# Wallacoloo/libfriendship

Hardware: AMD Instinct MI355X
Metric: Msamples/sec at 4096 partials x 64 voices; achieved HBM GB/s vs roofline (higher is better)
Workload: dtype f32

## Files before the change

libfriendship_amd/build.py:

```python
import os
import subprocess
import sys

PKG_DIR = os.path.dirname(os.path.abspath(__file__))
CSRC = os.path.join(PKG_DIR, "csrc")
OUT = os.path.join(PKG_DIR, "libfriendship_hip.so")
SOURCES = ["engine.cpp", "graph.cpp", "match.cpp", "stage.cpp", "jit.cpp", "leafjit.cpp", "stagejit.cpp", "comm_rccl.cpp", "kernels.hip"]
HEADERS = ["bankplan.hpp", "graph.hpp", "kernels.hpp", "match.hpp", "stage.hpp", "jit.hpp", "leafshape.hpp", "comm.hpp", "range.hpp", os.path.join("..", "..", "include", "friendship_render.h"),
           os.path.join("..", "..", "include", "friendship_render_ext.h")]
FLAGS = ["--offload-arch=gfx950", "-O3", "-std=c++17", "-fPIC", "-shared", "-ffp-contract=off",
         "-fno-slp-vectorize", "-mllvm", "-simplifycfg-sink-common=false", "-Wall", "-Wextra"]


def needs_build():
    if not os.path.exists(OUT):
        return True
    t = os.path.getmtime(OUT)
    deps = [os.path.join(CSRC, s) for s in SOURCES + HEADERS] + [os.path.abspath(__file__)]
    return any(os.path.getmtime(d) > t for d in deps)


def build(force=False, verbose=True):
    if not force and not needs_build():
        return OUT
    hipcc = os.environ.get("HIPCC", "/opt/rocm/bin/hipcc")
    cmd = [hipcc] + FLAGS + ["-o", OUT] + [os.path.join(CSRC, s) for s in SOURCES] + ["-lhiprtc", "-ldl"]
    if verbose:
        print(" ".join(cmd), file=sys.stderr)
    subprocess.run(cmd, check=True)
    return OUT


if __name__ == "__main__":
    build(force="--force" in sys.argv)
```

libfriendship_amd/csrc/engine.cpp:

```cpp
#include <hip/hip_runtime_api.h>

#include <algorithm>
#include <cfloat>
#include <cmath>
#include <cstdio>
#include <cstdlib>
#include <chrono>
#include <cstring>
#include <sstream>
#include <string>
#include <unordered_set>
#include <vector>

#include "../../include/friendship_render_ext.h"
#include "bankplan.hpp"
#include "comm.hpp"
#include "graph.hpp"
#include "jit.hpp"
#include "kernels.hpp"
#include "match.hpp"
#include "stage.hpp"

namespace fr {

// ... 14 lines not shown
    DevBuf(DevBuf &&o) noexcept : p(o.p), bytes(o.bytes) { o.p = nullptr; o.bytes = 0; }
    DevBuf &operator=(DevBuf &&o) noexcept {
        if (this != &o) { release(); p = o.p; bytes = o.bytes; o.p = nullptr; o.bytes = 0; }
        return *this;
    }
    ~DevBuf() { release(); }
    void release() {
        if (p) (void)hipFree(p);
        p = nullptr;
        bytes = 0;
    }
    void ensure(size_t n) {
        if (n <= bytes) return;
        release();
        size_t want = std::max(n, (size_t)256);
        HIP_CHECK(hipMalloc(&p, want));
        bytes = want;
    }
    template <class T> T *as() const { return (T *)p; }
};

struct PinnedBuf {
    void *p = nullptr;
    void *dev = nullptr;
    size_t bytes = 0;
    PinnedBuf() = default;
    PinnedBuf(const PinnedBuf &) = delete;
    PinnedBuf &operator=(const PinnedBuf &) = delete;
    ~PinnedBuf() { if (p) (void)hipHostFree(p); }
    void ensure(size_t n) {
        if (n <= bytes) return;
        if (p) (void)hipHostFree(p);
        p = dev = nullptr;
        bytes = 0;
        size_t want = std::max(n, (size_t)4096);
        HIP_CHECK(hipHostMalloc(&p, want, hipHostMallocMapped));
        HIP_CHECK(hipHostGetDevicePointer(&dev, p, 0));
        bytes = want;
    }
    template <class T> T *as() const { return (T *)p; }
    template <class T> T *as_dev() const { return (T *)dev; }
};

struct InSlot {
    bool fed = false;
    uint64_t base = 0;
    uint64_t len = 0;
    DevBuf buf;
    uint64_t cap = 0;
};

struct BankStage {
    BankLaunch grp;
    DevBuf d_params, d_rows, d_groups, d_group_off;
    std::shared_ptr<JitKernel> jit;
};

struct Plan {
    bool valid = false;
    uint64_t version = 0;
    uint64_t shard_epoch = 0;
    bool jit_pending = false;
    uint64_t jit_epoch = 0;
    uint32_t n_slots = 0;
    uint32_t max_depth = 0;
    std::vector<BankStage> banks;
    StagedPlan sp;
    DevBuf d_instrs, d_progs;
    std::shared_ptr<JitKernel> stage_jit;
    DevBuf d_jprogs, d_ptab;
    uint32_t stage_shapes = 0;
    bool stage_valid = false;
    uint64_t stage_end = 0;
    std::vector<uint32_t> pull_rows;
    DevBuf d_split_dst;
    DevBuf d_nodes, d_roots;
    std::vector<uint32_t> input_slots;
    const FlatGraph *graph = nullptr;
    bool observed_stale = false;
    std::string json;
};

struct BankLaunchNote {
    BankPlan launch;
    uint32_t voices, partials;
    uint64_t frames;
    uint32_t log2_p, leaf_variant;
    bool row_flags;
};

constexpr size_t N_OPTIONS = 29;

struct TimerClass {
    double ms = 0;
    uint64_t launches = 0;
    std::vector<std::pair<hipEvent_t, hipEvent_t>> pending;
};

__attribute__((weak)) hipError_t launch_input_range(const RangeArgs &a, hipStream_t) {
    for (uint32_t r = 0; r < a.n_rows; ++r)
        for (uint32_t b = 0; b < a.blocks; ++b) {
            RangePart o{HUGE_VALF, -HUGE_VALF, 0, 0};
            for (uint64_t i = (uint64_t)b * RANGE_THREADS; i < a.len[r]; i += (uint64_t)a.blocks * RANGE_THREADS)
                for (uint64_t j = i; j < std::min<uint64_t>(i + RANGE_THREADS, a.len[r]); ++j) {
                    const float v = a.row[r][j];
                    if (v != v) o.flags |= RANGE_NAN;
                    else if (v == HUGE_VALF) o.flags |= RANGE_POS_INF;
// ... 682 lines not shown
        Plan p;
        p.version = mirror.version;
        p.shard_epoch = shard_epoch;
        p.n_slots = n_slots;
        const ShardSpec *shard_spec = sharded() ? &shard : nullptr;
        const auto t_begin = std::chrono::steady_clock::now();
        uint32_t lower_lo = 0, lower_hi = UINT32_MAX;
        if (sharded() && shard.mode == FR_SHARD_VOICES) my_rows(n_slots, lower_lo, lower_hi);
        const FlatGraph &fg = lowering.update(mirror, n_slots, lower_lo, lower_hi, sharded() && shard.mode == FR_SHARD_PARTIALS);
        const double lower_ms = std::chrono::duration<double, std::milli>(std::chrono::steady_clock::now() - t_begin).count();
        p.max_depth = fg.max_depth;
        bool use_jit = allow_jit && mode == FR_MODE_AUTO;
        if (!matcher || matcher_gen != lowering.generation()) {
            matcher.reset(new BankMatcher(fg, 20, use_jit, allow_template, track_from));
            matcher_gen = lowering.generation();
        }
        p.graph = &fg;
        const ObservedInputs obs = observed_inputs(st);
        const ObservedInputs *observed = delay_observed ? &obs : nullptr;
        p.sp = plan_stages(fg, mode == FR_MODE_AUTO, mode != FR_MODE_PULL, 20, use_jit, allow_template, matcher.get(), shard_spec, track_from, observed, track_history);
        std::vector<std::shared_ptr<JitKernel>> jits(p.sp.banks.size());
        p.jit_epoch = jit_cache.epoch();
        if (use_jit) {
            bool without = false;
            try {
                for (size_t i = 0; i < p.sp.banks.size(); ++i)
                    if (p.sp.banks[i].jit) {
                        const bool wait = p.sp.banks[i].tracks && jit_async_configured;
                        if (wait) jit_cache.set_async(false);
                        struct Restore { JitCache &c; bool on; ~Restore() { if (on) c.set_async(true); } } restore{jit_cache, wait};
                        jits[i] = jit_cache.get(p.sp.banks[i].shape, p.sp.banks[i].varying, p.sp.banks[i].literal_bits, p.sp.banks[i].alias);
                        if (!jits[i]) p.jit_pending = without = true;
                    }
            } catch (const Error &e) {
                jit_error = e.what();
                without = true;
                if (sharded() && shard.mode == FR_SHARD_PARTIALS && e.code != FR_ERR_UNSUPPORTED)
                    throw Error(FR_ERR_DEVICE, std::string("a kernel of the sharded plan could not be compiled on this rank (every rank must plan alike): ") + e.what());
            }
            if (without) {
                p.sp = plan_stages(fg, true, true, 20, false, true, nullptr, shard_spec, track_from, observed, track_history);
                jits.assign(p.sp.banks.size(), nullptr);
            }
        }
        size_t bank_i = 0;
        for (BankLaunch &bg : p.sp.banks) {
            BankStage bs;
            bs.jit = jits[bank_i++];
            bs.grp = std::move(bg);
            bs.d_params.ensure(bs.grp.params.size() * sizeof(float));
            bs.d_rows.ensure(bs.grp.rows.size() * sizeof(uint32_t));
            HIP_CHECK(hipMemcpyAsync(bs.d_params.p, bs.grp.params.data(), bs.grp.params.size() * sizeof(float), hipMemcpyHostToDevice, st));
            HIP_CHECK(hipMemcpyAsync(bs.d_rows.p, bs.grp.rows.data(), bs.grp.rows.size() * sizeof(uint32_t), hipMemcpyHostToDevice, st));
            if (bs.grp.general) {
                bs.d_groups.ensure(bs.grp.groups.size() * sizeof(uint32_t));
                bs.d_group_off.ensure(bs.grp.group_off.size() * sizeof(uint32_t));
                HIP_CHECK(hipMemcpyAsync(bs.d_groups.p, bs.grp.groups.data(), bs.grp.groups.size() * sizeof(uint32_t), hipMemcpyHostToDevice, st));
                HIP_CHECK(hipMemcpyAsync(bs.d_group_off.p, bs.grp.group_off.data(), bs.grp.group_off.size() * sizeof(uint32_t), hipMemcpyHostToDevice, st));
            }
            p.banks.push_back(std::move(bs));
        }
        p.sp.banks.clear();
        if (!p.sp.split.empty()) {
            std::vector<uint32_t> dst(p.sp.split.size());
            for (size_t i = 0; i < dst.size(); ++i) dst[i] = p.sp.split[i].dst | (p.sp.split[i].to_ring ? 0x80000000u : 0u);
            p.d_split_dst.ensure(dst.size() * sizeof(uint32_t));
            HIP_CHECK(hipMemcpyAsync(p.d_split_dst.p, dst.data(), dst.size() * sizeof(uint32_t), hipMemcpyHostToDevice, st));
            HIP_CHECK(hipStreamSynchronize(st));
        }
        if (!p.sp.progs.empty()) {
            p.d_instrs.ensure(p.sp.instrs.size() * sizeof(StageInstr));
            p.d_progs.ensure(p.sp.progs.size() * sizeof(StageProg));
            HIP_CHECK(hipMemcpyAsync(p.d_instrs.p, p.sp.instrs.data(), p.sp.instrs.size() * sizeof(StageInstr), hipMemcpyHostToDevice, st));
            HIP_CHECK(hipMemcpyAsync(p.d_progs.p, p.sp.progs.data(), p.sp.progs.size() * sizeof(StageProg), hipMemcpyHostToDevice, st));
            StageJitPlan sj;
            if (allow_jit && stage_jit_mode != 0 && plan_stage_jit(p.sp.progs, p.sp.instrs, 32, stage_jit_mode == 2, sj, mirror.sparkle,
                                                                              stage_block_env ? stage_block_env : (p.sp.feedback ? 16u : 1u),
                                                                              p.sp.feedback && p.sp.fused_carry_only)) {
                try {
                    p.stage_jit = jit_cache.get_source(sj.source, "jit_stage");
                    if (!p.stage_jit) {
                        p.jit_pending = true;
                        throw Error(FR_OK, "");
                    }
                    p.stage_shapes = sj.n_shapes;
                    p.d_jprogs.ensure(sj.progs.size() * sizeof(JitStageProg));
                    p.d_ptab.ensure(std::max<size_t>(sj.ptab.size(), 1) * sizeof(uint32_t));
                    HIP_CHECK(hipMemcpyAsync(p.d_jprogs.p, sj.progs.data(), sj.progs.size() * sizeof(JitStageProg), hipMemcpyHostToDevice, st));
                    if (!sj.ptab.empty())
                        HIP_CHECK(hipMemcpyAsync(p.d_ptab.p, sj.ptab.data(), sj.ptab.size() * sizeof(uint32_t), hipMemcpyHostToDevice, st));
                    HIP_CHECK(hipStreamSynchronize(st));
                } catch (const Error &e) {
                    if (e.code != FR_OK) jit_error = e.what();
                    p.stage_jit = nullptr;
                }
            }
        }
        p.pull_rows = p.sp.pull_rows;
        if (!p.pull_rows.empty()) {
            std::vector<DevNode> dn(fg.nodes.size());
            std::unordered_map<uint32_t, uint32_t> dense;
            for (size_t i = 0; i < dn.size(); ++i) {
                const FlatNode &n = fg.nodes[i];
                dn[i] = DevNode{n.op, n.a, n.b, n.depth};
                if (n.op == OP_INPUT) {
                    auto it = dense.emplace(n.a, (uint32_t)p.input_slots.size());
// ... 252 lines not shown
                        d_chunk_rows.ensure(seq.size() * sizeof(uint32_t));
                        HIP_CHECK(hipMemcpyAsync(d_chunk_rows.p, seq.data(), seq.size() * sizeof(uint32_t), hipMemcpyHostToDevice, st));
                        HIP_CHECK(hipStreamSynchronize(st));
                        d_chunk_rows_n = (uint32_t)seq.size();
                    }
                    j.out = d_chunk_ws.as<float>();
                    j.rows = d_chunk_rows.as<uint32_t>();
                    j.out_stride = blen;
                }
                if (bs.grp.tracks && trk) {
                    j.tracks = trk->p;
                    j.track_stride = trk->stride;
                    j.track_limit = trk->limit;
                } else if (bs.grp.tracks && call_tracks) {
                    if (b0 != idx || blen != n_times) throw Error(FR_ERR_UNSUPPORTED, "internal: a voice that reads tracks rendered over another window than the call's");
                    j.tracks = call_tracks;
                    j.track_stride = call_track_stride;
                    j.track_limit = (uint32_t)std::min<uint64_t>((uint64_t)track_from + call_track_rows, 0xFFFFFFFFull);
                }
                note_bank_launch(bp, bs, blen, flag_out.host_flags != nullptr);
                Scope sc(this, &t_bank, st);
                HIP_CHECK(launch_jit_bank(*bs.jit, j, st));
                if (bp.pieces_log2) {
                    ChunkCombineArgs c{};
                    c.ws = d_chunk_ws.as<float>();
                    c.out = a.out;
                    c.rows = a.rows;
                    c.out_stride = a.out_stride;
                    c.n_times = blen;
                    c.n_voices = a.n_voices;
                    c.log2_c = bp.pieces_log2;
                    HIP_CHECK(launch_chunk_combine(c, st));
                }
                sc.done();
                return;
            }
            a.voices_per_wave = bp.voices_per_wave;
            if (bs.grp.general) {
                a.groups = bs.d_groups.as<uint32_t>();
                a.group_off = bs.d_group_off.as<uint32_t>();
                a.hist_dst = nullptr;
                note_bank_launch(bp, bs, blen, flag_out.host_flags != nullptr);
                Scope sc(this, &t_bank, st);
                HIP_CHECK(launch_gbank(a, st));
                sc.done();
                return;
            }
            if (a.hist_dst && !bp.appends_rows) throw Error(FR_ERR_DEVICE, "internal: deferred history append on a short call");
            a.chunk_log2 = bp.chunk_log2;
            a.frames_per_lane = bp.frames_per_lane;
            a.waves_per_group = bp.waves_per_group;
            a.small_call = bp.small_call;
            a.leaf_variant = bank_tune.leaf_variant;
            if (flag_out.host_flags) {
                if (!bp.publishes_rows) throw Error(FR_ERR_DEVICE, "internal: a bank launch cannot publish row flags");
                a.host_flags = flag_out.host_flags;
                a.row_done = flag_out.row_done;
                a.flag_value = flag_out.value;
            }
            if (bp.ws_floats) {
                used_scratch = true;
                d_bank_ws.ensure(bp.ws_floats * sizeof(float));
                a.ws = d_bank_ws.as<float>();
                if (bp.ticket_words) {
                    const size_t need = bp.ticket_words * sizeof(uint32_t);
                    clean_counters(st);
                    if (need > d_tickets.bytes) {
                        d_tickets.ensure(need * 2);
                        HIP_CHECK(hipMemsetAsync(d_tickets.p, 0, d_tickets.bytes, st));
                    }
                    a.tickets = d_tickets.as<uint32_t>();
                }
            }
            note_bank_launch(bp, bs, blen, flag_out.host_flags != nullptr);
            Scope sc(this, &t_bank, st);
            HIP_CHECK(launch_bank(a, st));
            sc.done();
        };
        auto launch_bank_window = [&](BankStage &bs, uint64_t b0, uint64_t blen, int64_t tile_off) {
            if (!(bs.grp.tracks && tail_on() && tile_off < 0 && b0 < idx && b0 + blen == idx + n_times)) {
                launch_bank_part(bs, b0, blen, tile_off, nullptr);
                return;
            }
            for (uint64_t s0 = b0; s0 < idx;) {
                const uint64_t pos = s0 & (tail_cap - 1);
                const uint64_t len = std::min(idx - s0, tail_cap - pos);
                TrackSrc ts{nullptr, tail_cap, 0};
                if (tail_rows) {
                    ts.p = reinterpret_cast<const float *>(reinterpret_cast<uintptr_t>(d_tail.as<float>() + pos) - (uintptr_t)track_from * tail_cap * sizeof(float));
                    ts.limit = (uint32_t)std::min<uint64_t>((uint64_t)track_from + tail_rows, 0xFFFFFFFFull);
                }
                launch_bank_part(bs, s0, len, -1, &ts);
                s0 += len;
            }
            launch_bank_part(bs, idx, n_times, -1, nullptr);
        };
        std::vector<DevInput> tab(sp.input_slots.size());
        auto fill_tab = [&] {
            for (size_t i = 0; i < tab.size(); ++i) tab[i] = dev_input(sp.input_slots[i]);
            if (tab.size() > STAGE_INLINE_INPUTS) {
                d_in_table_stage.ensure(tab.size() * sizeof(DevInput));
                HIP_CHECK(hipMemcpyAsync(d_in_table_stage.p, tab.data(), tab.size() * sizeof(DevInput), hipMemcpyHostToDevice, st));
                HIP_CHECK(hipStreamSynchronize(st));
            }
        };
        uint64_t launch_stride = 0;
// ... 922 lines not shown
```

libfriendship_amd/csrc/kernels.hip:

```cpp
#include <hip/hip_runtime.h>

#include <cstdlib>
#include <type_traits>

#include "kernels.hpp"

#pragma clang fp contract(off)

namespace fr {

#ifdef FR_DIAG_STAMPS
__device__ unsigned long long *g_diag = nullptr;
#define FR_DIAG_MARK(slot)                                                                                                 \
    do {                                                                                                                   \
        if (g_diag && (threadIdx.x & 63u) == 0u) {                                                                         \
            unsigned long long v_ = __builtin_amdgcn_s_memrealtime();                                                      \
            if ((slot) == 3) v_ = (unsigned long long)__builtin_amdgcn_s_getreg(0xF804) | ((unsigned long long)(__builtin_amdgcn_s_getreg(0xF814) & 15u) << 32); \
            g_diag[((size_t)blockIdx.x * 16u + (threadIdx.x >> 6)) * 8u + (slot)] = v_;                                    \
            if ((slot) != 3) g_diag[((size_t)blockIdx.x * 16u + (threadIdx.x >> 6)) * 8u + 4u + (slot)] = __builtin_amdgcn_s_memtime(); \
        }                                                                                                                  \
    } while (0)
#else
#define FR_DIAG_MARK(slot) do { } while (0)
#endif
// ... 134 lines not shown
    float w[8], A[8];
};

__device__ __forceinline__ void load_group(ParamGroup &pg, const_f32_ptr p, uint32_t g) {
#pragma unroll
    for (int j = 0; j < 8; ++j) {
        pg.w[j] = p[(size_t)g * 16 + 2 * j];
        pg.A[j] = p[(size_t)g * 16 + 2 * j + 1];
    }
}

template <int I, int N, class Fn>
__device__ __forceinline__ void static_for(Fn &&fn) {
    if constexpr (I < N) {
        fn(std::integral_constant<int, I>{});
        static_for<I + 1, N>(fn);
    }
}

template <int F>
using Lvl = float (&)[F];
#define FR_LEVELS_DECL Lvl<F> s0, Lvl<F> s1, Lvl<F> s2, Lvl<F> s3, Lvl<F> s4, Lvl<F> s5, Lvl<F> s6, Lvl<F> s7, Lvl<F> s8
#define FR_LEVELS_PASS s0, s1, s2, s3, s4, s5, s6, s7, s8

template <int F, bool FAST, bool EXACT>
__device__ __forceinline__ void bank_group(const ParamGroup &pg, uint32_t g,
                                           const float (&t)[F], FR_LEVELS_DECL) {
    float v[F];
#pragma unroll
    for (int f = 0; f < F; ++f) {
        float l0 = bank_leaf<FAST, EXACT>(t[f], pg.w[0], pg.A[0]);
        float l1 = bank_leaf<FAST, EXACT>(t[f], pg.w[1], pg.A[1]);
        float l2 = bank_leaf<FAST, EXACT>(t[f], pg.w[2], pg.A[2]);
        float l3 = bank_leaf<FAST, EXACT>(t[f], pg.w[3], pg.A[3]);
        float l4 = bank_leaf<FAST, EXACT>(t[f], pg.w[4], pg.A[4]);
        float l5 = bank_leaf<FAST, EXACT>(t[f], pg.w[5], pg.A[5]);
        float l6 = bank_leaf<FAST, EXACT>(t[f], pg.w[6], pg.A[6]);
        float l7 = bank_leaf<FAST, EXACT>(t[f], pg.w[7], pg.A[7]);
        v[f] = ((l0 + l1) + (l2 + l3)) + ((l4 + l5) + (l6 + l7));
    }
#define FR_CARRY(K, SK)                                                    \
    if (((g >> K) & 1u) == 0u) {       \
        static_for<0, F>([&](auto f) { SK[f] = v[f]; });                   \
        return;                                                            \
    }                                                                      \
    static_for<0, F>([&](auto f) { v[f] = SK[f] + v[f]; });
    FR_CARRY(0u, s0) FR_CARRY(1u, s1) FR_CARRY(2u, s2) FR_CARRY(3u, s3) FR_CARRY(4u, s4)
    FR_CARRY(5u, s5) FR_CARRY(6u, s6) FR_CARRY(7u, s7)
#undef FR_CARRY
#pragma unroll
    for (int f = 0; f < F; ++f) s8[f] = v[f];
}

template <int F, bool FAST, bool EXACT>
__device__ __forceinline__ void bank_wave_sum(const float *params, uint32_t ngroups, uint32_t levels,
                                              const float (&t)[F], float (&res)[F], const ParamGroup *first = nullptr) {
    float s0[F], s1[F], s2[F], s3[F], s4[F], s5[F], s6[F], s7[F], s8[F];
#pragma unroll
    for (int f = 0; f < F; ++f)
        s0[f] = s1[f] = s2[f] = s3[f] = s4[f] = s5[f] = s6[f] = s7[f] = s8[f] = 0.0f;

    const_f32_ptr p = (const_f32_ptr)params;
    ParamGroup pa, pb;
    if (first) pa = *first;
    else load_group(pa, p, 0);
    for (uint32_t g = 0; g < ngroups; g += 2) {
        const bool has_b = g + 1 < ngroups;
        __builtin_amdgcn_s_waitcnt(0xC07F);
        if (has_b) load_group(pb, p, g + 1);
        bank_group<F, FAST, EXACT>(pa, g, t, FR_LEVELS_PASS);
        if (has_b) {
            __builtin_amdgcn_s_waitcnt(0xC07F);
            if (g + 2 < ngroups) load_group(pa, p, g + 2);
            bank_group<F, FAST, EXACT>(pb, g + 1, t, FR_LEVELS_PASS);
        }
    }
#pragma unroll
    for (int f = 0; f < F; ++f) {
        float r = s8[f];
        r = levels == 7u ? s7[f] : r;
        r = levels == 6u ? s6[f] : r;
        r = levels == 5u ? s5[f] : r;
        r = levels == 4u ? s4[f] : r;
        r = levels == 3u ? s3[f] : r;
        r = levels == 2u ? s2[f] : r;
        r = levels == 1u ? s1[f] : r;
        r = levels == 0u ? s0[f] : r;
        res[f] = r;
    }
}

__device__ __forceinline__ bool leaves_all_negzero(const float2 *params, uint32_t n, float t, uint32_t tid, uint32_t nthreads) {
    bool ok = true;
    for (uint32_t k = tid; k < n && ok; k += nthreads) {
        float2 p = params[k];
        ok = __float_as_uint(bank_leaf<false, true>(t, p.x, p.y)) == 0x80000000u;
    }
    return ok;
}

template <bool FAST>
__device__ __attribute__((noinline)) bool wave_leaves_all_negzero(const float *params, uint32_t ngroups, float t, unsigned long long lanes) {
    const_f32_ptr p = (const_f32_ptr)params;
    const bool wanted = (lanes >> (threadIdx.x & 63u)) & 1ull;
    uint32_t all_and = 0xFFFFFFFFu, all_or = 0u;
    ParamGroup pa, pb;
    load_group(pa, p, 0);
    auto fold = [&](const ParamGroup &pg) {
#pragma unroll
        for (int j = 0; j < 8; ++j) {
            uint32_t b = __float_as_uint(bank_leaf<FAST, true>(t, pg.w[j], pg.A[j]));
            all_and &= b;
            all_or |= b;
        }
    };
    for (uint32_t g = 0; g < ngroups; g += 2) {
        const bool has_b = g + 1 < ngroups;
        __builtin_amdgcn_s_waitcnt(0xC07F);
        if (has_b) load_group(pb, p, g + 1);
        fold(pa);
        if (has_b) {
            __builtin_amdgcn_s_waitcnt(0xC07F);
            if (g + 2 < ngroups) load_group(pa, p, g + 2);
            fold(pb);
        }
        if (__ballot(wanted && all_and == 0x80000000u && all_or == 0x80000000u) == 0ull) {
            __builtin_amdgcn_s_waitcnt(0xC07F);
            return false;
        }
    }
    return all_and == 0x80000000u && all_or == 0x80000000u;
}

__device__ __forceinline__ float bank_time(const BankArgs &a, uint64_t ti) {
    return (ti >= a.time_skip && ti - a.time_skip < a.time_valid) ? a.time[ti - a.time_skip] : 0.0f;
}
__device__ __forceinline__ uint64_t bank_out_index(const BankArgs &a, uint64_t ti) {
    return a.ring_mask ? ((a.ring_t0 + ti) & a.ring_mask) : ti;
}

template <int F, int MODE, int NW, bool FLAGS = false>
__global__ void __launch_bounds__(64 * NW) bank_kernel(BankArgs a, uint32_t tiles, uint32_t nblocks) {
    uint32_t b = blockIdx.x;
    uint32_t lid = (nblocks % 8u == 0u) ? (b % 8u) * (nblocks / 8u) + b / 8u : b;
    const uint32_t nchunks = 1u << (a.log2_p - a.chunk_log2);
    const uint32_t vc = lid / tiles;
    const uint32_t tile = lid - vc * tiles;
    const uint32_t voice = vc >> (a.log2_p - a.chunk_log2);
    const uint32_t chunk = vc & (nchunks - 1u);
    const uint32_t lane = threadIdx.x & 63u;
    const uint32_t wave = __builtin_amdgcn_readfirstlane(threadIdx.x >> 6);

    FR_DIAG_MARK(0);
    FR_DIAG_MARK(3);
    const uint64_t t0 = (uint64_t)tile * (64u * F);
    float t[F];
    bool nonneg = true;
#pragma unroll
    for (int f = 0; f < F; ++f) {
        uint64_t ti = t0 + (uint32_t)f * 64u + lane;
        t[f] = bank_time(a, ti);
        nonneg = nonneg && (t[f] >= 0.0f) && (t[f] <= 4294967296.0f);
        if (a.hist_dst && vc == 0u && wave == 0u && ti < a.time_valid) a.hist_dst[ti] = t[f];
    }
    const bool fast = a.fast_ok && __all(nonneg);

    const uint32_t Pc = 1u << a.chunk_log2;
    const uint32_t Pw = Pc / NW;
    const float2 *cparams = a.params + ((size_t)voice << a.log2_p) + (size_t)chunk * Pc;
    const float *params = (const float *)(cparams + (size_t)wave * Pw);
    const uint32_t ngroups = Pw >> 3;
    const uint32_t levels = a.chunk_log2 - 3u - (NW == 8 ? 3u : NW == 4 ? 2u : NW == 2 ? 1u : 0u);

    float res[F];
    constexpr bool EXACT = (MODE == 0);
    if (fast) bank_wave_sum<F, true, EXACT>(params, ngroups, levels, t, res);
    else bank_wave_sum<F, false, EXACT>(params, ngroups, levels, t, res);
    FR_DIAG_MARK(1);

    __shared__ float sm[NW][F][64];
    __shared__ unsigned long long zmask[F];
#pragma unroll
    for (int f = 0; f < F; ++f) sm[wave][f][lane] = res[f];
    __syncthreads();
    FR_DIAG_MARK(2);
    const bool direct = nchunks == 1u;
    float *orow = direct ? a.out + (size_t)a.rows[voice] * a.out_stride
                         : a.ws + ((size_t)chunk * a.n_voices + voice) * a.n_times;
    if (wave == 0) {
#pragma unroll
        for (int f = 0; f < F; ++f) {
            uint64_t ti = t0 + (uint32_t)f * 64u + lane;
            float r = sm[0][f][lane];
            if (NW >= 2) r = r + sm[1 % NW][f][lane];
            if (NW >= 4) r = r + (sm[2 % NW][f][lane] + sm[3 % NW][f][lane]);
            if (NW == 8) r = r + ((sm[4 % NW][f][lane] + sm[5 % NW][f][lane]) + (sm[6 % NW][f][lane] + sm[7 % NW][f][lane]));
            bool live = ti < a.n_times;
            if (live) {
                float *dst = &orow[direct ? bank_out_index(a, ti) : ti];
                if (FLAGS) __hip_atomic_store(dst, r, __ATOMIC_RELAXED, __HIP_MEMORY_SCOPE_SYSTEM);
                else __builtin_nontemporal_store(r, dst);
            }
            if (MODE == 1) {
                unsigned long long m = __ballot(live && r == 0.0f);
                if (lane == 0) zmask[f] = m;
            }
        }
    }
    if (MODE == 1) {
        __syncthreads();
#pragma unroll
        for (int f = 0; f < F; ++f) {
            unsigned long long m = zmask[f];
            if (__builtin_popcountll(m) > 4) {
                bool mine = fast ? wave_leaves_all_negzero<true>(params, ngroups, t[f], m)
                                 : wave_leaves_all_negzero<false>(params, ngroups, t[f], m);
                sm[wave][f][lane] = mine ? 1.0f : 0.0f;
                __syncthreads();
                if (wave == 0 && ((m >> lane) & 1ull)) {
                    bool all = true;
#pragma unroll
                    for (int w = 0; w < NW; ++w) all = all && sm[w][f][lane] != 0.0f;
                    uint64_t ti = t0 + (uint32_t)f * 64u + lane;
                    float *dst = &orow[direct ? bank_out_index(a, ti) : ti];
                    if (FLAGS) __hip_atomic_store(dst, all ? -0.0f : 0.0f, __ATOMIC_RELAXED, __HIP_MEMORY_SCOPE_SYSTEM);
                    else *dst = all ? -0.0f : 0.0f;
                }
                __syncthreads();
                continue;
            }
            while (m) {
                uint32_t l = (uint32_t)__builtin_ctzll(m);
                m &= m - 1;
                uint64_t ti = t0 + (uint32_t)f * 64u + l;
                float tz = bank_time(a, ti);
                int all = __syncthreads_and(leaves_all_negzero(cparams, Pc, tz, threadIdx.x, 64u * NW) ? 1 : 0);
                if (threadIdx.x == 0) {
                    float *dst = &orow[direct ? bank_out_index(a, ti) : ti];
                    if (FLAGS) __hip_atomic_store(dst, all ? -0.0f : 0.0f, __ATOMIC_RELAXED, __HIP_MEMORY_SCOPE_SYSTEM);
                    else *dst = all ? -0.0f : 0.0f;
                }
            }
        }
    }
    if (FLAGS && a.host_flags && direct && wave == 0) {
        asm volatile("s_waitcnt vmcnt(0)" ::: "memory");
        if (lane == 0u) {
            const uint32_t old = __hip_atomic_fetch_add(a.row_done + voice, 1u, __ATOMIC_RELAXED, __HIP_MEMORY_SCOPE_AGENT);
            if (old == tiles - 1u) {
// ... 1038 lines not shown
```

libfriendship_amd/csrc/kernels.hpp:

```cpp
#pragma once

#include <hip/hip_runtime_api.h>

#include <cstdint>

namespace fr {

struct DevInput {
    const float *data;
    uint64_t base;
    uint64_t len;
};

struct DevNode {
    uint32_t op, a, b, depth;
};

struct PullArgs {
    const DevNode *nodes;
    const uint32_t *outputs;
    const DevInput *inputs;
    uint32_t n_inputs;
    float *out;
    uint32_t n_slots;
    uint64_t n_times;
    uint64_t idx;
    uint64_t first;
    uint64_t count;
    uint32_t sparkle;
    uint32_t *st_node;
    uint64_t *st_time;
    float *st_val;
};
hipError_t launch_pull(const PullArgs &a, hipStream_t s);

struct BankArgs {
    const float2 *params;
    const float *time;
    uint64_t time_skip;
    uint64_t time_valid;
    float *out;
    const uint32_t *rows;
    uint64_t out_stride;
    uint64_t ring_mask;
    uint64_t ring_t0;
    uint32_t n_voices;
    uint32_t log2_p;
    uint64_t n_times;
    uint32_t fast_ok;
    uint32_t chunk_log2;
    uint32_t frames_per_lane;
    uint32_t waves_per_group;
    uint32_t small_call;
    uint32_t voices_per_wave;
    uint32_t leaf_variant;
    float *hist_dst;
    float *ws;
    uint32_t *row_done;
    uint32_t *host_flags;
    uint32_t flag_value;
    uint32_t *tickets;
    const uint32_t *groups;
    const uint32_t *group_off;
};
constexpr uint32_t BANK_TICKET_STRIDE = 32;

struct BankStreamCtl {
    unsigned long long row[64];
    uint32_t done;
    uint32_t alive;
    uint32_t pad1[14];
};
struct BankStreamDev {
    uint32_t seq;
    uint32_t n_times;
    uint32_t voices_done;
    uint32_t pad[13];
    float row[64];
};
constexpr uint32_t BANK_STREAM_STOP = 0xFFFFFFFFu;
constexpr uint32_t BANK_STREAM_WGS = 256;
constexpr uint32_t BANK_STREAM_IDLE_MS = 2000;
hipError_t launch_bank_stream(const BankArgs &a, BankStreamCtl *ctl_dev, BankStreamDev *dev, uint32_t idle_ms, hipStream_t s);
uint64_t bank_blocks(const BankArgs &a);
hipError_t launch_bank(const BankArgs &a, hipStream_t s);
hipError_t launch_gbank(const BankArgs &a, hipStream_t s);

enum StageOp : uint8_t {
    S_CONST = 0,
    S_INPUT = 1,
    S_READ = 2,
    S_READ_INPUT = 3,
    S_STEP = 4,
    S_SUM2 = 5, S_MUL = 6, S_DIV = 7, S_MOD = 8, S_MIN = 9,
    S_STORE = 10,
    S_READ_DYN = 11,
    S_READ_INPUT_DYN = 12,
    S_STEP_DYN = 13,
};
struct StageInstr {
    uint8_t op, dst, a, b;
    uint32_t imm;
    uint32_t buf;
    uint32_t d_lo;
};
struct StageProg {
    uint32_t first_instr, n_instr;
    uint32_t result_reg;
    uint32_t dst_ring;
    int32_t out_row;
    uint32_t n_loads;
    uint32_t pad[2];
};
constexpr int STAGE_REGS = 48;
constexpr uint32_t STAGE_INLINE_INPUTS = 8;
constexpr uint32_t STAGE_MAX_HOISTED = 24;
// ... 89 lines not shown
```

libfriendship_amd/csrc/stage.cpp:

```cpp
#include "stage.hpp"

#include "range.hpp"

#include <algorithm>
#include <cmath>
#include <memory>
#include <string>
#include <unordered_map>
#include <unordered_set>

#include <chrono>
#include <cstdio>
#include <cstdlib>
namespace fr {
namespace {
struct PlanTrace {
    bool on = std::getenv("FR_PLAN_TRACE") != nullptr;
    std::chrono::steady_clock::time_point t = std::chrono::steady_clock::now();
    void mark(const char *what) {
        if (!on) return;
        auto n = std::chrono::steady_clock::now();
        std::fprintf(stderr, "  plan_stages: -> %s after %.3f ms\n", what, std::chrono::duration<double, std::milli>(n - t).count());
        t = n;
    }
};
#define FR_PT(x) plan_trace.mark(x)

constexpr uint32_t NO_RING = 0xFFFFFFFFu;
constexpr size_t MAX_PROG_INSTR = 4096;
constexpr uint64_t FUSED_UNBOUNDED = 1ull << 31;

struct Planner {
    const FlatGraph &g;
    BankMatcher *matcher;
    std::unordered_map<uint32_t, int8_t> supported_memo;
    std::unordered_map<uint32_t, const VoiceMatch *> bank_of;
    std::unordered_set<uint32_t> cut;
    std::unordered_set<uint32_t> visited;

    Planner(const FlatGraph &fg, BankMatcher *m) : g(fg), matcher(m) {}

    static bool delay_frames_ok(const FlatGraph &g, const FlatNode &n, uint64_t &frames) {
        if (!g.is_const(n.b)) return false;
        float d = g.const_val(n.b);
        if (!(d >= 1.0f) || d >= 2147483648.0f) return false;
        frames = (uint64_t)d;
        return true;
    }

    using Range = fr::Range;
    std::unordered_map<uint32_t, Range> range_memo, obs_memo;
    std::unordered_map<uint32_t, uint64_t> dyn_max;
    const ObservedInputs *observed = nullptr;
    std::unordered_set<uint32_t> observed_dyn;
// ... 112 lines not shown
                if (1 + sa + sb <= limit) { size[n] = 1 + sa + sb; break; }
                uint32_t big = (!delay && sa >= sb) ? x.a : x.b;
                if (size[big] <= 1) { size[n] = 1 + sa + sb; break; }
                cut.insert(big);
                size[big] = 1;
            }
        }
    }

    void explore(uint32_t root) {
        std::vector<uint32_t> st{root};
        while (!st.empty()) {
            uint32_t n = st.back();
            st.pop_back();
            if (is_leaf(n) || !visited.insert(n).second) continue;
            const FlatNode &x = g.nodes[n];
            if (is_voice(n)) continue;
            if (x.op == OP_DELAY) {
                const uint32_t src = g.src_of(x.a);
                if (!is_leaf(src)) cut.insert(src);
                st.push_back(src);
                if (dyn_max.count(n)) st.push_back(x.b);
            } else {
                st.push_back(x.a);
                st.push_back(x.b);
            }
        }
    }
};

std::string voice_key(const VoiceMatch &vm, bool ring, bool ws) {
    std::string key = std::to_string(vm.general ? 63u : vm.log2_p) + "/" + std::to_string(vm.input_slot) + (vm.general ? "g" : "") + (ring ? "r" : "") + (ws ? "w" : "");
    if (vm.jit) {
        key += "j" + vm.shape.key();
        for (uint32_t sl : vm.shape.input_slots) key += "s" + std::to_string(sl);
        for (size_t c = 0; c < vm.varying.size(); ++c)
            key += vm.varying[c] ? ("v" + std::to_string(vm.alias[c])) : ("l" + std::to_string(vm.literal_bits[c]));
    }
    return key;
}

void add_voice(std::vector<BankLaunch> &banks, std::unordered_map<std::string, size_t> &grp, const VoiceMatch &vm, uint32_t row, bool ring,
               bool ws = false, const std::unordered_map<std::string, size_t> *totals = nullptr) {
    const std::string key = voice_key(vm, ring, ws);
    auto gi = grp.find(key);
    if (gi == grp.end()) {
        gi = grp.emplace(key, banks.size()).first;
        BankLaunch bl;
        bl.log2_p = vm.log2_p; bl.input_slot = vm.input_slot; bl.to_ring = ring; bl.to_ws = ws; bl.general = vm.general;
        if (vm.general) { bl.group_off.push_back(0); bl.group_off.push_back(0); }
        if (vm.jit) { bl.jit = true; bl.shape = vm.shape; bl.varying = vm.varying; bl.literal_bits = vm.literal_bits; bl.alias = vm.alias; bl.k = vm.k; bl.tracks = vm.tracks; }
        if (totals) {
            auto ti = totals->find(key);
            if (ti != totals->end()) bl.params.reserve(ti->second);
        }
        banks.push_back(std::move(bl));
    }
    BankLaunch &bl = banks[gi->second];
    bl.rows.push_back(row);
    bl.params.insert(bl.params.end(), vm.params.begin(), vm.params.end());
    bl.fast_ok = bl.fast_ok && vm.fast_ok;
    bl.max_track_slot = std::max(bl.max_track_slot, vm.max_track_slot);
    if (vm.general) {
        bl.groups.insert(bl.groups.end(), vm.groups.begin(), vm.groups.end());
        bl.group_off.push_back((uint32_t)bl.groups.size());
        bl.group_off.push_back((uint32_t)(bl.params.size() / 16));
        bl.max_leaves = std::max(bl.max_leaves, vm.n_leaves);
    }
}

struct ProgBuild {
    std::vector<StageInstr> instrs;
    uint32_t result_reg = 0;
    uint32_t n_loads = 0;
    std::vector<std::pair<uint32_t, uint64_t>> reads;
    std::unordered_set<uint32_t> dynamic_reads;
};

bool build_program(const FlatGraph &g, const Planner &P, uint32_t m, std::unordered_map<uint32_t, uint32_t> &dense_input,
                   std::vector<uint32_t> &input_slots, ProgBuild &out, bool fuse = false,
                   const std::unordered_set<uint32_t> *stored = nullptr, uint64_t *min_delay = nullptr, uint64_t *gcd_delay = nullptr) {
    auto is_boundary = [&](uint32_t n) {
        if (n == m) return false;
        if (P.bank_of.count(n)) return true;
        return !fuse && P.cut.count(n) != 0;
    };
    std::vector<uint32_t> order;
    std::unordered_map<uint32_t, uint32_t> uses;
    {
        std::unordered_set<uint32_t> seen;
        std::vector<std::pair<uint32_t, int>> st{{m, 0}};
        while (!st.empty()) {
            auto [n, state] = st.back();
            st.pop_back();
            if (state == 1) { order.push_back(n); continue; }
            if (!seen.insert(n).second) continue;
            st.push_back({n, 1});
            const FlatNode &x = g.nodes[n];
            if (is_boundary(n) || x.op == OP_CONST || x.op == OP_INPUT) continue;
            if (x.op == OP_DELAY) {
                if (P.dyn_max.count(n)) { ++uses[x.b]; st.push_back({x.b, 0}); }
                continue;
            }
            ++uses[x.a];
            ++uses[x.b];
            st.push_back({x.b, 0});
            st.push_back({x.a, 0});
        }
    }
    {
        auto is_load = [&](uint32_t n) {
            const FlatNode &x = g.nodes[n];
            return is_boundary(n) || x.op == OP_CONST || x.op == OP_INPUT || (x.op == OP_DELAY && !P.dyn_max.count(n));
// ... 800 lines not shown
```

libfriendship_amd/csrc/stage.hpp:

```cpp
#pragma once

#include <algorithm>
#include <cstdint>
#include <functional>
#include <memory>
#include <vector>

#include "graph.hpp"
#include "kernels.hpp"
#include "match.hpp"
#include "range.hpp"

namespace fr {

struct BankLaunch {
    uint32_t log2_p = 0;
    uint32_t input_slot = 0;
    bool fast_ok = true;
    bool to_ring = false;
    bool to_ws = false;
    std::vector<uint32_t> rows;
    std::vector<float> params;
    bool general = false;
    std::vector<uint32_t> groups;
    std::vector<uint32_t> group_off;
    uint32_t max_leaves = 0;
    bool jit = false;
    LeafShape shape;
    std::vector<bool> varying;
    std::vector<uint32_t> literal_bits;
    std::vector<uint32_t> alias;
    uint32_t k = 0;
    bool tracks = false;
    uint32_t max_track_slot = 0;
};

struct ShardSpec {
    uint32_t rank = 0, world = 1;
    int mode = FR_SHARD_NONE;
};
inline void shard_row_range(uint32_t rank, uint32_t world, uint32_t n_rows, uint32_t &lo, uint32_t &hi) {
    const uint32_t q = n_rows / world, r = n_rows % world;
    lo = rank * q + std::min(rank, r);
    hi = lo + q + (rank < r ? 1u : 0u);
}
inline uint32_t shard_row_owner(uint32_t row, uint32_t world, uint32_t n_rows) {
    const uint32_t q = n_rows / world, r = n_rows % world;
    const uint32_t big = r * (q + 1);
    return row < big ? row / (q + 1) : r + (q ? (row - big) / q : 0);
}

struct SplitVoice {
    uint32_t owner = 0;
    bool to_ring = false;
    uint32_t dst = 0;
};

struct StagedPlan {
    std::vector<BankLaunch> banks;
    std::vector<SplitVoice> split;
    std::vector<StageInstr> instrs;
    std::vector<StageProg> progs;
    std::vector<uint32_t> level_first;
    uint32_t fused_first = 0, fused_count = 0;
    uint64_t fused_max_frames = 0;
    uint64_t fused_stride = 0;
    bool feedback = false;
    uint32_t feedback_loops = 0;
    std::vector<uint32_t> fused_level_first;
    uint32_t post_first = 0, post_count = 0;
    bool fused_carry_only = false;
    uint32_t n_rings = 0;
    uint64_t lmax = 0;
    uint64_t input_lookback = 0;
    bool input_lookback_unbounded = false;
// ... 27 lines not shown
```

Before: 40.53.

## Skip saturated partial groups in bank kernel using precomputed saturation times

At plan time, a per-group saturation time is computed on the host for each group of 8 partials. It is the earliest time at which the phase product reaches a threshold, after which those partials presumably contribute a fixed or negligible value. The bank kernel uses this table with ballot and popcount to count the live prefix of groups for the current time tile. It then sums only those groups, redistributes the remaining blocks across waves with a tree reduction in shared memory, and changes the voice-chunk block ordering and launch bounds. This is meant to cut parameter reads and arithmetic for partials that no longer need evaluating, at the cost of extra host precomputation, a small device table, and more complex reduction logic that could change the summation order.

```diff
diff --git a/libfriendship_amd/build.py b/libfriendship_amd/build.py
--- a/libfriendship_amd/build.py
+++ b/libfriendship_amd/build.py
@@ -6,7 +6,7 @@
 CSRC = os.path.join(PKG_DIR, "csrc")
 OUT = os.path.join(PKG_DIR, "libfriendship_hip.so")
 SOURCES = ["engine.cpp", "graph.cpp", "match.cpp", "stage.cpp", "jit.cpp", "leafjit.cpp", "stagejit.cpp", "comm_rccl.cpp", "kernels.hip"]
-HEADERS = ["bankplan.hpp", "graph.hpp", "kernels.hpp", "match.hpp", "stage.hpp", "jit.hpp", "leafshape.hpp", "comm.hpp", "range.hpp", os.path.join("..", "..", "include", "friendship_render.h"),
+HEADERS = ["bankplan.hpp", "banksat.hpp", "graph.hpp", "kernels.hpp", "match.hpp", "stage.hpp", "jit.hpp", "leafshape.hpp", "comm.hpp", "range.hpp", os.path.join("..", "..", "include", "friendship_render.h"),
            os.path.join("..", "..", "include", "friendship_render_ext.h")]
 FLAGS = ["--offload-arch=gfx950", "-O3", "-std=c++17", "-fPIC", "-shared", "-ffp-contract=off",
          "-fno-slp-vectorize", "-mllvm", "-simplifycfg-sink-common=false", "-Wall", "-Wextra"]
diff --git a/libfriendship_amd/csrc/banksat.hpp b/libfriendship_amd/csrc/banksat.hpp
--- /dev/null
+++ b/libfriendship_amd/csrc/banksat.hpp
@@ -0,0 +1,37 @@
+#pragma once
+
+#include <algorithm>
+#include <cmath>
+#include <cstddef>
+#include <cstdint>
+#include <vector>
+
+namespace fr {
+
+constexpr float BANK_SAT_PHASE = 4194304.0f;
+constexpr float BANK_SAT_TMAX = 4294967296.0f;
+
+inline float bank_sat_time(float s) {
+    const float inf = INFINITY;
+    if (!(s > 0.0f) || !(s <= BANK_SAT_TMAX) || !(BANK_SAT_TMAX * s >= BANK_SAT_PHASE)) return inf;
+    float t = std::min(BANK_SAT_PHASE / s, BANK_SAT_TMAX);
+    while (t > 0.0f && std::nextafterf(t, 0.0f) * s >= BANK_SAT_PHASE) t = std::nextafterf(t, 0.0f);
+    while (t * s < BANK_SAT_PHASE) t = std::nextafterf(t, inf);
+    return t;
+}
+
+inline float bank_sat_w(float w, float a4) {
+    return (w >= 0.0f && w <= BANK_SAT_TMAX && std::isfinite(a4)) ? w : 0.0f;
+}
+
+inline void bank_sat_append(std::vector<float> &out, const float *params, size_t P) {
+    const size_t G = (P + 7) / 8, base = out.size();
+    out.resize(base + G);
+    float s = INFINITY;
+    for (size_t g = G; g-- > 0;) {
+        for (size_t k = std::min(P, 8 * g + 8); k-- > 8 * g;) s = std::min(s, bank_sat_w(params[2 * k], params[2 * k + 1]));
+        out[base + g] = bank_sat_time(s);
+    }
+}
+
+}
diff --git a/libfriendship_amd/csrc/engine.cpp b/libfriendship_amd/csrc/engine.cpp
--- a/libfriendship_amd/csrc/engine.cpp
+++ b/libfriendship_amd/csrc/engine.cpp
@@ -90,7 +90,7 @@
 
 struct BankStage {
     BankLaunch grp;
-    DevBuf d_params, d_rows, d_groups, d_group_off;
+    DevBuf d_params, d_rows, d_groups, d_group_off, d_t_sat;
     std::shared_ptr<JitKernel> jit;
 };
 
@@ -879,6 +879,10 @@
             bs.d_rows.ensure(bs.grp.rows.size() * sizeof(uint32_t));
             HIP_CHECK(hipMemcpyAsync(bs.d_params.p, bs.grp.params.data(), bs.grp.params.size() * sizeof(float), hipMemcpyHostToDevice, st));
             HIP_CHECK(hipMemcpyAsync(bs.d_rows.p, bs.grp.rows.data(), bs.grp.rows.size() * sizeof(uint32_t), hipMemcpyHostToDevice, st));
+            if (!bs.grp.t_sat.empty()) {
+                bs.d_t_sat.ensure(bs.grp.t_sat.size() * sizeof(float));
+                HIP_CHECK(hipMemcpyAsync(bs.d_t_sat.p, bs.grp.t_sat.data(), bs.grp.t_sat.size() * sizeof(float), hipMemcpyHostToDevice, st));
+            }
             if (bs.grp.general) {
                 bs.d_groups.ensure(bs.grp.groups.size() * sizeof(uint32_t));
                 bs.d_group_off.ensure(bs.grp.group_off.size() * sizeof(uint32_t));
@@ -1237,6 +1241,7 @@
             a.waves_per_group = bp.waves_per_group;
             a.small_call = bp.small_call;
             a.leaf_variant = bank_tune.leaf_variant;
+            a.t_sat = bs.d_t_sat.as<float>();
             if (flag_out.host_flags) {
                 if (!bp.publishes_rows) throw Error(FR_ERR_DEVICE, "internal: a bank launch cannot publish row flags");
                 a.host_flags = flag_out.host_flags;
diff --git a/libfriendship_amd/csrc/kernels.hip b/libfriendship_amd/csrc/kernels.hip
--- a/libfriendship_amd/csrc/kernels.hip
+++ b/libfriendship_amd/csrc/kernels.hip
@@ -210,7 +210,7 @@
     for (int f = 0; f < F; ++f) s8[f] = v[f];
 }
 
-template <int F, bool FAST, bool EXACT>
+template <int F, bool FAST, bool EXACT, bool PREFIX = false>
 __device__ __forceinline__ void bank_wave_sum(const float *params, uint32_t ngroups, uint32_t levels,
                                               const float (&t)[F], float (&res)[F], const ParamGroup *first = nullptr) {
     float s0[F], s1[F], s2[F], s3[F], s4[F], s5[F], s6[F], s7[F], s8[F];
@@ -233,6 +233,18 @@
             bank_group<F, FAST, EXACT>(pb, g + 1, t, FR_LEVELS_PASS);
         }
     }
+    if (PREFIX && ngroups != (1u << levels)) {
+        bool have = false;
+#define FR_FOLD(K, SK)                                                                                   \
+        if ((ngroups >> K) & 1u) {                                                                       \
+            static_for<0, F>([&](auto f) { res[f] = have ? SK[f] + res[f] : SK[f]; });                   \
+            have = true;                                                                                 \
+        }
+        FR_FOLD(0u, s0) FR_FOLD(1u, s1) FR_FOLD(2u, s2) FR_FOLD(3u, s3) FR_FOLD(4u, s4)
+        FR_FOLD(5u, s5) FR_FOLD(6u, s6) FR_FOLD(7u, s7)
+#undef FR_FOLD
+        return;
+    }
 #pragma unroll
     for (int f = 0; f < F; ++f) {
         float r = s8[f];
@@ -297,13 +309,29 @@
     return a.ring_mask ? ((a.ring_t0 + ti) & a.ring_mask) : ti;
 }
 
+__device__ __forceinline__ uint32_t bank_live_seg(uint32_t ng) { return (ng + 63u) >> 6; }
+__device__ __forceinline__ float bank_live_first(const float *ts, uint32_t ng, uint32_t lane) {
+    const uint32_t seg = bank_live_seg(ng);
+    return ts[min((lane + 1u) * seg, ng) - 1u];
+}
+__device__ __forceinline__ uint32_t bank_live_groups(const float *ts, uint32_t ng, float end, float tmin, uint32_t lane) {
+    const uint32_t seg = bank_live_seg(ng), nseg = (ng + seg - 1u) / seg;
+    const uint32_t c = (uint32_t)__builtin_popcountll(__ballot(lane < nseg && end > tmin));
+    if (c == nseg) return ng;
+    const uint32_t g = c * seg + lane;
+    const bool live = lane < seg && g < ng && ts[min(g, ng - 1u)] > tmin;
+    return c * seg + (uint32_t)__builtin_popcountll(__ballot(live));
+}
+
 template <int F, int MODE, int NW, bool FLAGS = false>
-__global__ void __launch_bounds__(64 * NW) bank_kernel(BankArgs a, uint32_t tiles, uint32_t nblocks) {
+__global__ void __launch_bounds__(64 * NW, (MODE == 1 && F == 1) ? 8 : 1) bank_kernel(BankArgs a, uint32_t tiles, uint32_t nblocks) {
     uint32_t b = blockIdx.x;
     uint32_t lid = (nblocks % 8u == 0u) ? (b % 8u) * (nblocks / 8u) + b / 8u : b;
     const uint32_t nchunks = 1u << (a.log2_p - a.chunk_log2);
-    const uint32_t vc = lid / tiles;
+    uint32_t vc = lid / tiles;
     const uint32_t tile = lid - vc * tiles;
+    const uint32_t nvc = a.n_voices * nchunks;
+    if (MODE == 1 && a.t_sat && nblocks % 8u == 0u && nvc % 8u == 0u) vc = (vc % 8u) * (nvc / 8u) + vc / 8u;
     const uint32_t voice = vc >> (a.log2_p - a.chunk_log2);
     const uint32_t chunk = vc & (nchunks - 1u);
     const uint32_t lane = threadIdx.x & 63u;
@@ -311,20 +339,27 @@
 
     FR_DIAG_MARK(0);
     FR_DIAG_MARK(3);
+    const uint32_t Pc = 1u << a.chunk_log2;
+    const uint32_t Pw = Pc / NW;
+    const uint32_t NG = Pc >> 3;
+    const bool skip = MODE == 1 && a.t_sat != nullptr;
+    const float *ts = skip ? a.t_sat + ((size_t)voice << (a.log2_p - 3u)) + (size_t)chunk * NG : nullptr;
+    const float ts_end = skip ? bank_live_first(ts, NG, lane) : 0.0f;
     const uint64_t t0 = (uint64_t)tile * (64u * F);
     float t[F];
+#pragma unroll
+    for (int f = 0; f < F; ++f) t[f] = bank_time(a, t0 + (uint32_t)f * 64u + lane);
     bool nonneg = true;
+    float tmin = INFINITY;
 #pragma unroll
     for (int f = 0; f < F; ++f) {
         uint64_t ti = t0 + (uint32_t)f * 64u + lane;
-        t[f] = bank_time(a, ti);
         nonneg = nonneg && (t[f] >= 0.0f) && (t[f] <= 4294967296.0f);
+        if (ti < a.n_times) tmin = fminf(tmin, t[f]);
         if (a.hist_dst && vc == 0u && wave == 0u && ti < a.time_valid) a.hist_dst[ti] = t[f];
     }
     const bool fast = a.fast_ok && __all(nonneg);
 
-    const uint32_t Pc = 1u << a.chunk_log2;
-    const uint32_t Pw = Pc / NW;
     const float2 *cparams = a.params + ((size_t)voice << a.log2_p) + (size_t)chunk * Pc;
     const float *params = (const float *)(cparams + (size_t)wave * Pw);
     const uint32_t ngroups = Pw >> 3;
@@ -332,14 +367,47 @@
 
     float res[F];
     constexpr bool EXACT = (MODE == 0);
-    if (fast) bank_wave_sum<F, true, EXACT>(params, ngroups, levels, t, res);
-    else bank_wave_sum<F, false, EXACT>(params, ngroups, levels, t, res);
+    constexpr uint32_t NBMAX = MODE == 1 ? (16 / F > NW ? 16 / F : NW) : NW;
+    __shared__ float sm[NBMAX][F][64];
+    __shared__ unsigned long long zmask[F];
+    uint32_t nb = NW;
+    if constexpr (MODE == 1) {
+        uint32_t L = NG;
+        if (skip && fast) {
+            const uint32_t m = __ockl_wfred_min_u32(__float_as_uint(tmin));
+            L = bank_live_groups(ts, NG, ts_end, __uint_as_float(__builtin_amdgcn_readfirstlane(m)), lane);
+        }
+        uint32_t h = levels, k0 = wave, k1 = wave + 1u;
+        if (L != NG) {
+            uint32_t best = 0xFFFFFFFFu;
+            for (uint32_t hh = levels + 1u; hh-- > 0u;) {
+                const uint32_t n = (L + (1u << hh) - 1u) >> hh;
+                if (n > NBMAX) break;
+                const uint32_t per = (n + NW - 1u) / NW;
+                const uint32_t cost = min(per << hh, L) + per;
+                if (cost < best) { best = cost; h = hh; }
+            }
+            nb = (L + (1u << h) - 1u) >> h;
+            const uint32_t q = nb / NW, rem = nb % NW;
+            const uint32_t w2 = rem ? (wave + lid) % NW : wave;
+            k0 = w2 * q + min(w2, rem);
+            k1 = k0 + q + (w2 < rem ? 1u : 0u);
+        }
+        for (uint32_t k = k0; k < k1; ++k) {
+            const float *bp = (const float *)(cparams + ((size_t)k << (h + 3u)));
+            const uint32_t G = min(1u << h, L - (k << h));
+            if (fast) bank_wave_sum<F, true, EXACT, true>(bp, G, h, t, res);
+            else bank_wave_sum<F, false, EXACT, true>(bp, G, h, t, res);
+#pragma unroll
+            for (int f = 0; f < F; ++f) sm[k][f][lane] = res[f];
+        }
+    } else {
+        if (fast) bank_wave_sum<F, true, EXACT>(params, ngroups, levels, t, res);
+        else bank_wave_sum<F, false, EXACT>(params, ngroups, levels, t, res);
+#pragma unroll
+        for (int f = 0; f < F; ++f) sm[wave][f][lane] = res[f];
+    }
     FR_DIAG_MARK(1);
-
-    __shared__ float sm[NW][F][64];
-    __shared__ unsigned long long zmask[F];
-#pragma unroll
-    for (int f = 0; f < F; ++f) sm[wave][f][lane] = res[f];
     __syncthreads();
     FR_DIAG_MARK(2);
     const bool direct = nchunks == 1u;
@@ -349,10 +417,19 @@
 #pragma unroll
         for (int f = 0; f < F; ++f) {
             uint64_t ti = t0 + (uint32_t)f * 64u + lane;
-            float r = sm[0][f][lane];
-            if (NW >= 2) r = r + sm[1 % NW][f][lane];
-            if (NW >= 4) r = r + (sm[2 % NW][f][lane] + sm[3 % NW][f][lane]);
-            if (NW == 8) r = r + ((sm[4 % NW][f][lane] + sm[5 % NW][f][lane]) + (sm[6 % NW][f][lane] + sm[7 % NW][f][lane]));
+            float r;
+            if (nb == NW) {
+                r = sm[0][f][lane];
+                if (NW >= 2) r = r + sm[1 % NW][f][lane];
+                if (NW >= 4) r = r + (sm[2 % NW][f][lane] + sm[3 % NW][f][lane]);
+                if (NW == 8) r = r + ((sm[4 % NW][f][lane] + sm[5 % NW][f][lane]) + (sm[6 % NW][f][lane] + sm[7 % NW][f][lane]));
+            } else {
+                for (uint32_t n = nb; n > 1u; n = (n + 1u) >> 1) {
+                    for (uint32_t k = 0; 2u * k + 1u < n; ++k) sm[k][f][lane] = sm[2u * k][f][lane] + sm[2u * k + 1u][f][lane];
+                    if (n & 1u) sm[n >> 1][f][lane] = sm[n - 1u][f][lane];
+                }
+                r = nb ? sm[0][f][lane] : 0.0f;
+            }
             bool live = ti < a.n_times;
             if (live) {
                 float *dst = &orow[direct ? bank_out_index(a, ti) : ti];
diff --git a/libfriendship_amd/csrc/kernels.hpp b/libfriendship_amd/csrc/kernels.hpp
--- a/libfriendship_amd/csrc/kernels.hpp
+++ b/libfriendship_amd/csrc/kernels.hpp
@@ -62,6 +62,7 @@
     uint32_t *tickets;
     const uint32_t *groups;
     const uint32_t *group_off;
+    const float *t_sat;
 };
 constexpr uint32_t BANK_TICKET_STRIDE = 32;
 
diff --git a/libfriendship_amd/csrc/stage.cpp b/libfriendship_amd/csrc/stage.cpp
--- a/libfriendship_amd/csrc/stage.cpp
+++ b/libfriendship_amd/csrc/stage.cpp
@@ -1,5 +1,6 @@
 #include "stage.hpp"
 
+#include "banksat.hpp"
 #include "range.hpp"
 
 #include <algorithm>
@@ -218,13 +219,17 @@
         if (vm.jit) { bl.jit = true; bl.shape = vm.shape; bl.varying = vm.varying; bl.literal_bits = vm.literal_bits; bl.alias = vm.alias; bl.k = vm.k; bl.tracks = vm.tracks; }
         if (totals) {
             auto ti = totals->find(key);
-            if (ti != totals->end()) bl.params.reserve(ti->second);
+            if (ti != totals->end()) {
+                bl.params.reserve(ti->second);
+                if (!vm.general && !vm.jit) bl.t_sat.reserve(ti->second / 16);
+            }
         }
         banks.push_back(std::move(bl));
     }
     BankLaunch &bl = banks[gi->second];
     bl.rows.push_back(row);
     bl.params.insert(bl.params.end(), vm.params.begin(), vm.params.end());
+    if (!vm.general && !vm.jit) bank_sat_append(bl.t_sat, vm.params.data(), vm.params.size() / 2);
     bl.fast_ok = bl.fast_ok && vm.fast_ok;
     bl.max_track_slot = std::max(bl.max_track_slot, vm.max_track_slot);
     if (vm.general) {
diff --git a/libfriendship_amd/csrc/stage.hpp b/libfriendship_amd/csrc/stage.hpp
--- a/libfriendship_amd/csrc/stage.hpp
+++ b/libfriendship_amd/csrc/stage.hpp
@@ -21,6 +21,7 @@
     bool to_ws = false;
     std::vector<uint32_t> rows;
     std::vector<float> params;
+    std::vector<float> t_sat;
     bool general = false;
     std::vector<uint32_t> groups;
     std::vector<uint32_t> group_off;
```

Measured after the change: 40.13, median of 2. 0.99x the previous value.
